# 0xPabloxx/3d-pointcloud-orientation-estimation

Hardware: AMD Instinct MI355X
Metric: clouds/sec fwd+bwd, pointnet_pp_vonMises N=1024 (higher is better)
Workload: dtype f32; 1 GPU; configs[1]: models/pointnet_pp_vonMises.py single-peak KL, N=1024, batch=32 per GPU, fwd+loss+bwd+allreduce+Adam, random-init weights (seed 42), device-side centre sampling; per_gpu_batch=32, global_batch=32, points=1024, parallelism=single, launch=hipGraph(fwd+loss+bwd) + eager all-reduce/Adam (the update clears the gradients)

## Files before the change

### 3d-pointcloud-orientation-estimation_amd/csrc/dw_kernels.hip

```cpp
#include "gemm_smallm.h"
#include "launch.h"
#include "split_prims.h"

namespace pnpp {

template <int DZMODE, int A2MODE, int CT, int KT>
__global__ void __launch_bounds__(256)
dw_kernel(const AOperand dz, const AOperand a2, int M, int Nc, int Kp, int tilesC, int tilesK, int rows_per_split,
          int kp_pad, float *__restrict__ slab, int policy) {
    constexpr int U = 4;
    const int lane = threadIdx.x & 63, l31 = lane & 31, lh = lane >> 5;
    const int gw = blockIdx.x * 4 + (threadIdx.x >> 6);
    const int tiles = tilesC * tilesK;
    const int tile = gw % tiles, split = gw / tiles;
    const int r0 = min(M, split * rows_per_split);
    const int r1 = min(M, r0 + rows_per_split);
    const int c0 = (tile % tilesC) * 32 * CT, k0 = (tile / tilesC) * 32 * KT;

    ChanConst cc[CT], ck[KT];
#pragma unroll
    for (int i = 0; i < CT; ++i) cc[i] = load_chan_const<DZMODE>(dz, c0 + i * 32 + l31, Nc);
#pragma unroll
    for (int j = 0; j < KT; ++j) ck[j] = load_chan_const<A2MODE>(a2, k0 + j * 32 + l31, Kp);

// ... 330 lines not shown
__device__ __forceinline__ void dw_lds_tail(float *__restrict__ o, const f32x16 (&acc)[2][2], int cb, int kb, int Nc, int kp_pad) {
#pragma unroll
    for (int i = 0; i < 2; ++i)
#pragma unroll
        for (int j = 0; j < 2; ++j) {
            const int k = kb + j * 32;
#pragma unroll
            for (int r = 0; r < 16; ++r) {
                const int c = cb + i * 32 + (r & 3) + 8 * (r >> 2);
                if (c < Nc && k < kp_pad) sp_store(o + (size_t)c * kp_pad + k, acc[i][j][r], WT);
            }
        }
}

template <int DZMODE, int A2MODE, bool POLICY>
__device__ __forceinline__ void dw_lds_body(const AOperand &dz, const AOperand &a2, int M, int Nc, int Kp, int tilesC, int tilesK, int rps,
                                            int kp_pad, float *__restrict__ slab, int bx, const bool wt_dw) {
    __shared__ __attribute__((aligned(16))) float Dz[32][128];
    __shared__ __attribute__((aligned(16))) float A2[32][128];
    const int tid = threadIdx.x, lane = tid & 63, wave = __builtin_amdgcn_readfirstlane(tid >> 6);
    const int l31 = lane & 31, lh = lane >> 5;
    const int tiles = tilesC * tilesK;
    const int tile = bx % tiles, split = bx / tiles;
    const int c0 = (tile % tilesC) * 128, k0 = (tile / tilesC) * 128;
    const int r0 = min(M, split * rps), r1 = min(M, r0 + rps);
    const int wc = wave >> 1, wk = wave & 1;
    const int q4 = 4 * (tid & 31), rb = tid >> 5;

    f32x16 acc[2][2];
#pragma unroll
    for (int i = 0; i < 2; ++i)
#pragma unroll
        for (int j = 0; j < 2; ++j)
#pragma unroll
            for (int r = 0; r < 16; ++r) acc[i][j][r] = 0.f;

    RawA nd[4], na[4];
    auto fetch = [&](int m0) {
#pragma unroll
        for (int i = 0; i < 4; ++i) {
            nd[i] = fetch_a4<DZMODE>(dz, m0 + rb + 8 * i, c0 + q4, r1, Nc);
            na[i] = fetch_a4<A2MODE>(a2, m0 + rb + 8 * i, k0 + q4, r1, Kp);
        }
    };
    if (r0 < r1) fetch(r0);
    for (int m0 = r0; m0 < r1; m0 += 32) {
        __syncthreads();
#pragma unroll
        for (int i = 0; i < 4; ++i) {
            float v[4];
            xform_a4<DZMODE>(dz, nd[i], m0 + rb + 8 * i, c0 + q4, r1, Nc, v);
            *reinterpret_cast<float4 *>(&Dz[rb + 8 * i][q4]) = make_float4(v[0], v[1], v[2], v[3]);
            xform_a4<A2MODE>(a2, na[i], m0 + rb + 8 * i, k0 + q4, r1, Kp, v);
            *reinterpret_cast<float4 *>(&A2[rb + 8 * i][q4]) = make_float4(v[0], v[1], v[2], v[3]);
        }
        __syncthreads();
        if (m0 + 32 < r1) fetch(m0 + 32);
        const float *pd = &Dz[lh][wc * 64 + l31], *pa = &A2[lh][wk * 64 + l31];
#pragma unroll 4
        for (int rp = 0; rp < 16; ++rp) {
            const float d0 = pd[rp * 256], d1 = pd[rp * 256 + 32], b0 = pa[rp * 256], b1 = pa[rp * 256 + 32];
            acc[0][0] = __builtin_amdgcn_mfma_f32_32x32x2f32(d0, b0, acc[0][0], 0, 0, 0);
            acc[0][1] = __builtin_amdgcn_mfma_f32_32x32x2f32(d0, b1, acc[0][1], 0, 0, 0);
            acc[1][0] = __builtin_amdgcn_mfma_f32_32x32x2f32(d1, b0, acc[1][0], 0, 0, 0);
            acc[1][1] = __builtin_amdgcn_mfma_f32_32x32x2f32(d1, b1, acc[1][1], 0, 0, 0);
        }
    }
    float *o = slab + (size_t)split * Nc * kp_pad;
    if constexpr (POLICY) {
        if (wt_dw) dw_lds_tail<true>(o, acc, c0 + wc * 64 + 4 * lh, k0 + wk * 64 + l31, Nc, kp_pad);
        else dw_lds_tail<false>(o, acc, c0 + wc * 64 + 4 * lh, k0 + wk * 64 + l31, Nc, kp_pad);
    } else {
        dw_lds_tail<false>(o, acc, c0 + wc * 64 + 4 * lh, k0 + wk * 64 + l31, Nc, kp_pad);
    }
}

template <int DZMODE, int A2MODE>
__global__ void __launch_bounds__(256)
dw_lds_kernel(const AOperand dz, const AOperand a2, int M, int Nc, int Kp, int tilesC, int tilesK, int rps, int kp_pad,
              float *__restrict__ slab) {
    dw_lds_body<DZMODE, A2MODE, false>(dz, a2, M, Nc, Kp, tilesC, tilesK, rps, kp_pad, slab, blockIdx.x, false);
}

template <int EMODE, int A2MODE>
__global__ void __launch_bounds__(256)
da_dw_kernel(const AOperand dzA, const BOperand W, int M, int Nout, int Kd, const Epilogue E, int g1x, int g1, const AOperand a2, int Nc,
             int Kp, int tilesC, int tilesK, int rps, int kp_pad, float *__restrict__ slab) {
    if ((int)blockIdx.x < g1)
        gemm_smallm_body<A_PLAIN, EMODE, false, 4>(dzA, W, M, Nout, Kd, E, blockIdx.x % g1x, blockIdx.x / g1x, g1);
    else
        dw_lds_body<A_PLAIN, A2MODE, true>(dzA, a2, M, Nc, Kp, tilesC, tilesK, rps, kp_pad, slab, blockIdx.x - g1, (E.store_policy & ST_DW_SLABS) != 0);
}

void dw_plan(int M, int Nc, int Kp, int *nsplit, int *kp_pad) {
    const int tilesC = cdiv(Nc, 64), tilesK = cdiv(Kp, 64);
    const int tiles = tilesC * tilesK;
    int split = cdiv(2048, tiles);
    const int max_split = cdiv(M, M <= 4096 ? 32 : 64);
    if (split > max_split) split = max_split;
    if (split > 1024) split = 1024;
    if (split < 1) split = 1;
    *nsplit = split;
    *kp_pad = tilesK * 64;
}

int launch_dw(const AOperand &dz, int Nc, const AOperand &a2, int Kp, int M, float *slab, int nsplit, int kp_pad,
              hipStream_t st) {
    PNPP_REQUIRE(M > 0 && Nc > 0 && Kp > 0 && nsplit > 0, PNPP_ERR_ARG, "dw: non-positive size");
    const int tilesC = cdiv(Nc, 64), tilesK = cdiv(Kp, 64);
    PNPP_REQUIRE(kp_pad == tilesK * 64, PNPP_ERR_ARG, "dw: kp_pad mismatch");
    int rps = cdiv(M, nsplit);
    rps = (rps + 7) & ~7;
    if (M <= 4096 && Nc >= 128 && Kp >= 128 && dz.mode == A_PLAIN && (dz.lda & 3) == 0 && ((uintptr_t)dz.a & 15) == 0 &&
        (a2.mode == A_PLAIN || a2.mode == A_BNRELU || a2.mode == A_CONCAT) &&
        (a2.mode == A_CONCAT || ((a2.lda & 3) == 0 && ((uintptr_t)a2.a & 15) == 0))) {
        const int tc = cdiv(Nc, 128), tk = cdiv(Kp, 128);
        const dim3 grid(tc * tk * nsplit);
        ProfScope ps(st, "dw_lds_kernel<A%d,A%d> M=%d N=%d K=%d split=%d grid=%d", dz.mode, a2.mode, M, Nc, Kp, nsplit, grid.x);
        switch (a2.mode) {
            case A_PLAIN:
                hipLaunchKernelGGL((dw_lds_kernel<A_PLAIN, A_PLAIN>), grid, dim3(256), 0, st, dz, a2, M, Nc, Kp, tc, tk, rps, kp_pad, slab);
                break;
            case A_BNRELU:
                hipLaunchKernelGGL((dw_lds_kernel<A_PLAIN, A_BNRELU>), grid, dim3(256), 0, st, dz, a2, M, Nc, Kp, tc, tk, rps, kp_pad, slab);
                break;
            default:
                hipLaunchKernelGGL((dw_lds_kernel<A_PLAIN, A_CONCAT>), grid, dim3(256), 0, st, dz, a2, M, Nc, Kp, tc, tk, rps, kp_pad, slab);
                break;
        }
        PNPP_CHECK_LAUNCH("dw(lds)");
        return PNPP_OK;
    }
    const int waves = tilesC * tilesK * nsplit;
    const dim3 grid(cdiv(waves, 4)), block(256);
    ProfScope ps(st, "dw_kernel<A%d,A%d> M=%d N=%d K=%d split=%d grid=%dx1", dz.mode, a2.mode, M, Nc, Kp, nsplit, grid.x);
#define PNPP_DW(DM, AM)                                                                                              \
    hipLaunchKernelGGL((dw_kernel<DM, AM, 2, 2>), grid, block, 0, st, dz, a2, M, Nc, Kp, tilesC, tilesK, rps, kp_pad, slab, store_policy()); \
    break;
#define PNPP_DW_BY_A(DM)                         \
    switch (a2.mode) {                           \
        case A_PLAIN: PNPP_DW(DM, A_PLAIN)       \
        case A_BNRELU: PNPP_DW(DM, A_BNRELU)     \
        case A_GATHER: PNPP_DW(DM, A_GATHER)     \
        case A_CONCAT: PNPP_DW(DM, A_CONCAT)     \
        default: set_error("dw: bad A2 mode %d", a2.mode); return PNPP_ERR_ARG; \
    }                                            \
    break;
    switch (dz.mode) {
        case A_PLAIN: PNPP_DW_BY_A(A_PLAIN)
        case A_DZ: PNPP_DW_BY_A(A_DZ)
        case A_DZ_POOL: PNPP_DW_BY_A(A_DZ_POOL)
        default: set_error("dw: bad dZ mode %d", dz.mode); return PNPP_ERR_ARG;
    }
#undef PNPP_DW_BY_A
#undef PNPP_DW
    PNPP_CHECK_LAUNCH("dw");
    return PNPP_OK;
}

bool try_launch_da_dw(const AOperand &dz, const BOperand &Win, int M, int Nout, int Kd, const Epilogue &Ein, int *nslab, const AOperand &a2,
                      int Kp, float *slab, int *nsplit_io, int *kp_pad_io, hipStream_t st, int *rc, float *dw_direct, int dw_ld) {
    *rc = PNPP_OK;
    Epilogue E = Ein;
    E.store_policy = store_policy();
    if (mid_tiles_on() && try_launch_mid_da_dw(dz, Win, M, Nout, Kd, E, nslab, a2, Kp, slab, nsplit_io, kp_pad_io, st, rc, dw_direct, dw_ld))
        return true;
    const int nsplit = *nsplit_io, kp_pad = *kp_pad_io;
    const int Nc = Kd;
    if (!(M > 32 && M <= 4096 && cdiv(M, 32) <= kMaxStatBlocks && dz.mode == A_PLAIN && (dz.lda & 3) == 0 && ((uintptr_t)dz.a & 15) == 0))
        return false;
    if (!(Nc >= 128 && Kp >= 128 && Kd % 4 == 0 && !Win.trans && (E.mode == E_STORE || E.mode == E_MASK_STATS))) return false;
    if (!(a2.mode == A_PLAIN || a2.mode == A_BNRELU || a2.mode == A_CONCAT)) return false;
    if (a2.mode != A_CONCAT && ((a2.lda & 3) != 0 || ((uintptr_t)a2.a & 15) != 0)) return false;
    if (kp_pad != cdiv(Kp, 64) * 64 || nsplit < 1) return false;
    BOperand W = Win;
    if (W.rows <= 0 || W.rows > Kd) W.rows = Kd;
    const int g1x = cdiv(Nout, 32), g1y = cdiv(M, 32), g1 = g1x * g1y;
    const int tc = cdiv(Nc, 128), tk = cdiv(Kp, 128);
    int rps = cdiv(M, nsplit);
    rps = (rps + 7) & ~7;
    const dim3 grid(g1 + tc * tk * nsplit);
    if (nslab) *nslab = g1y;
    ProfScope ps(st, "da_dw_kernel<E%d,A%d> M=%d | dA N=%d K=%d grid=%d | dW N=%d K=%d split=%d grid=%d", E.mode, a2.mode, M, Nout, Kd, g1,
                 Nc, Kp, nsplit, tc * tk * nsplit);
#define PNPP_DADW(EM, AM) \
    hipLaunchKernelGGL((da_dw_kernel<EM, AM>), grid, dim3(256), 0, st, dz, W, M, Nout, Kd, E, g1x, g1, a2, Nc, Kp, tc, tk, rps, kp_pad, slab)
    if (E.mode == E_STORE) {
        if (a2.mode == A_PLAIN) PNPP_DADW(E_STORE, A_PLAIN);
        else if (a2.mode == A_BNRELU) PNPP_DADW(E_STORE, A_BNRELU);
        else PNPP_DADW(E_STORE, A_CONCAT);
    } else {
        if (a2.mode == A_PLAIN) PNPP_DADW(E_MASK_STATS, A_PLAIN);
        else if (a2.mode == A_BNRELU) PNPP_DADW(E_MASK_STATS, A_BNRELU);
        else PNPP_DADW(E_MASK_STATS, A_CONCAT);
    }
#undef PNPP_DADW
    check_launch("da_dw", rc);
    return true;
}

}
```

### 3d-pointcloud-orientation-estimation_amd/csrc/kernels.h

```cpp
#pragma once
#include "common.h"

namespace pnpp {

int launch_knn(const float *new_xyz, const float *xyz, int B, int S, int N, int k, int32_t *idx, hipStream_t st,
               const int32_t *lengths = nullptr);
int launch_knn_centres(const float *xyz, const int32_t *centre, int B, int S, int N, int k, int32_t *idx, float *out_a,
                       float *out_b, hipStream_t st, const int32_t *lengths = nullptr);
int launch_knn_pair(const float *xyz, int B, int N, const int32_t *centre1, int S1, int k1, int32_t *idx1, float *a1, float *b1,
                    const int32_t *centre2, int S2, int k2, int32_t *idx2, float *a2, float *b2, double *mom, hipStream_t st,
                    const int32_t *lengths = nullptr);
int knn_pair_moment_partials(int B, int S1, int N);
size_t knn_pair_moment_doubles(int B, int S1, int N);
int launch_gather_centres(const float *xyz, const int32_t *centre, int B, int N, int S, float *out_a, float *out_b, hipStream_t st);
int launch_scatter_rows_bwd(const float *dout, const int32_t *idx, int B, int N, int C, int M, float *dpoints, hipStream_t st);

enum AMode {
    A_PLAIN = 0,
    A_BNRELU = 1,
    A_GATHER = 2,
    A_CONCAT = 3,
    A_DZ = 4,
    A_DZ_POOL = 5
};
// ... 33 lines not shown
    unsigned long long *rng_counter = nullptr;
    int relu = 0;
    float *y = nullptr;
};

struct Epilogue {
    int mode = E_STORE;
    float *c = nullptr;
    int ldc = 0;
    double *slab = nullptr;
    const float *zp = nullptr;
    const float *scale = nullptr, *shift = nullptr, *mu = nullptr, *istd = nullptr;
    float *dwslab = nullptr;
    int dw_ld = 0;
    float *pool_ext = nullptr;
    int32_t *pool_arg = nullptr;
    const float *pool_gamma = nullptr;
    int store_policy = 0;
    BnTail bn;
};

struct BOperand {
    const float *b = nullptr;
    int ldb = 0;
    int trans = 0;
    int perm_D = -1;
    int rows = 0;
};

struct BnLayer {
    int C = 0;
    const float *bias = nullptr, *gamma = nullptr, *beta = nullptr;
    float *rm = nullptr, *rv = nullptr, *mean = nullptr, *istd = nullptr, *scale = nullptr, *shift = nullptr;
    long long *nbt = nullptr;
};
struct BnGrads { float *dgamma = nullptr, *dbeta = nullptr, *dbias = nullptr; };
struct BnHyper { float momentum = 0.1f, eps = 1e-5f; int training = 0; };
struct StatsView {
    const double *slab = nullptr;
    int nslab = 0;
    const double *count_dev = nullptr, *local = nullptr;
};
struct PoolTail {
    const float *pool_ext = nullptr;
    float *pool_out = nullptr;
    int32_t *pool_arg = nullptr;
    float *origin_a = nullptr, *origin_b = nullptr;
    int G = 0, norigin = 0;
};
struct DzSide { const AOperand *dz = nullptr; int M = 0; float *out = nullptr; };
struct SlabReduceArgs {
    const float *slab;
    int nsplit, Nc, kp_pad, Kvalid, perm_D;
    float *out;
    int ldo;
};

int launch_gemm(const AOperand &A, const BOperand &B, int M, int Nout, int Kd, const Epilogue &E, int *nslab,
                hipStream_t st, int *dw_slabs = nullptr);
bool mid_tiles_on();
bool try_launch_ws(const AOperand &A, const BOperand &B, int M, int Nout, int Kd, const Epilogue &E, int *nslab, hipStream_t st, int *rc,
                   int *dw_slabs);

int matmul_precision();
void set_matmul_precision(int bf16);
bool try_launch_ws_bf16(const AOperand &A, const BOperand &B, int M, int Nout, int Kd, const Epilogue &E, int *nslab, hipStream_t st,
                        int *rc, int *dw_slabs);

int launch_dw(const AOperand &dz, int Nc, const AOperand &a2, int Kp, int M, float *slab, int nsplit, int kp_pad,
              hipStream_t st);
int launch_dz_materialize(const AOperand &dz, int M, int C, float *out, hipStream_t st);
void dw_plan(int M, int Nc, int Kp, int *nsplit, int *kp_pad);
bool delayed_layer0_ok(int C);
int launch_gather_rel_stats(const float *P, const AOperand &geo, const float *W0, int ldw, int M, int C, float *z,
                            double *slab, int *nslab, hipStream_t st);
int scatter_dz_splits(int rows);
int launch_scatter_dz(const AOperand &dz, const AOperand &geo, int B, int Mc, int C, float *G, float *wslab, hipStream_t st);
int dw_xyz_splits(int M);
int launch_dw_xyz(const AOperand &dz, int Nc, const AOperand &a2, int M, float *slab, hipStream_t st);
bool try_launch_fc_dx_dw(const float *dz, const float *w, const float *x, int M, int N, int K, float *dx, float *dw, hipStream_t st,
                         int *rc);
bool try_launch_da_dw(const AOperand &dz, const BOperand &W, int M, int Nout, int Kd, const Epilogue &E, int *nslab, const AOperand &a2,
                      int Kp, float *slab, int *nsplit, int *kp_pad, hipStream_t st, int *rc, float *dw_direct = nullptr, int dw_ld = 0);
bool try_launch_mid_gemm(const AOperand &A, const BOperand &B, int M, int Nout, int Kd, const Epilogue &E, int *nslab, hipStream_t st,
                         int *rc);
bool mid_gemm_pools(const AOperand &A, int M, int Nout, int Kd);
bool try_launch_wsf(const AOperand &A, const BOperand &B, int M, int Nout, int Kd, const Epilogue &E, int *nslab, hipStream_t st, int *rc);
bool wsf_applies(const AOperand &A, const BOperand &B, int M, int Nout, int Kd, const Epilogue &E);
int split_products();
void set_split_products(int on);
int store_policy();
void set_store_policy(int mask);
bool try_launch_wsf3(const AOperand &A, const BOperand &B, int M, int Nout, int Kd, const Epilogue &E, int *nslab, hipStream_t st, int *rc);
bool try_launch_wsd3(const AOperand &A, const BOperand &B, int M, int Nout, int Kd, const Epilogue &E, int *nslab, hipStream_t st, int *rc,
                     int *dw_slabs);
int wsd3_timeouts();
bool try_launch_wsp(const AOperand &A, const BOperand &B, int M, int Nout, int Kd, const Epilogue &E, int *nslab, hipStream_t st, int *rc,
                    int *dw_slabs);
bool try_launch_wsq(const AOperand &A, const BOperand &B, int M, int Nout, int Kd, const Epilogue &E, int *nslab, hipStream_t st, int *rc,
                    int *dw_slabs);
bool try_launch_wsx(const AOperand &dz, const BOperand &W, int M, int C1, int C0, const AOperand &geo, const float *W0, int ldw0,
                    const float *scale0, const float *shift0, float *dwslab, double *stat, int *workers_out, hipStream_t st, int *rc);
size_t wsx_stat_doubles();
bool xyz0_applies(int M, int D, int K, int group_all, int L, const int *C);
size_t xyz0_moment_doubles();
int launch_rel_moments(const AOperand &geo, int M, double *mom, int *nmom, hipStream_t st);
int launch_wsf0(const AOperand &geo, int M, const BOperand &W0, const double *mom, int nmom, const BnLayer &bn0, const BnHyper &h,
                const BOperand &W1, const Epilogue &E, int *nslab, hipStream_t st);
int launch_xyz0_post(const SlabReduceArgs &R1, const double *stat, const BOperand &W0, const BnLayer &bn0, double count, int training,
                     float *dW0, int ld0, const BnGrads &g0, hipStream_t st);
int launch_relu_mask(const float *z, const float *scale, const float *shift, size_t n, int C, uint8_t *out, hipStream_t st);
int launch_xyz0_mask(const AOperand &geo, int M, const float *W0, int ldw0, const float *scale0, const float *shift0, uint8_t *out,
                     hipStream_t st);
unsigned wsx_build_flags();
unsigned wsf_build_flags();
unsigned wsd3_build_flags();
unsigned mid3_build_flags();
unsigned wsp_build_flags();
unsigned wsq_build_flags();
unsigned gemm_build_flags();
unsigned fc_build_flags();
bool try_launch_mid_da_dw(const AOperand &dz, const BOperand &W, int M, int Nout, int Kd, const Epilogue &E, int *nslab, const AOperand &a2,
                          int Kp, float *slab, int *nsplit_out, int *kp_pad_out, hipStream_t st, int *rc, float *dw_direct = nullptr,
                          int dw_ld = 0);
int launch_slab_reduce2(const float *slab1, int nsplit1, int Nc1, int kp_pad1, int Kvalid1, float *out1, int ldo1, const float *slab2,
                        int nsplit2, int Nc2, int kp_pad2, int Kvalid2, float *out2, int ldo2, hipStream_t st);
int launch_slab_reduce(const float *slab, int nsplit, int Nc, int kp_pad, int Kvalid, int perm_D, float *out, int ldo,
                       hipStream_t st);

int launch_bn_finalize_fwd(const StatsView &V, double count, const BnLayer &bn, const BnHyper &h, hipStream_t st,
                           const PoolTail *tail = nullptr);
bool gemm_pools_in_epilogue(const AOperand &A, int M, int Nout, int Kd, int nsample);
struct PooledSource {
    const float *dout = nullptr, *zsel = nullptr, *scale = nullptr, *shift = nullptr;
    int G = 0;
};
int launch_bn_finalize_bwd(const StatsView &V, double count, int training, const BnLayer &bn, float *cst, const BnGrads &g, hipStream_t st,
                           const DzSide &dz = DzSide(), const PooledSource *pooled = nullptr);
int launch_post_gemm(const StatsView &V, double count, int training, const BnLayer &bn, float *cst, const BnGrads &g, const SlabReduceArgs &R,
                     hipStream_t st, const DzSide &dz = DzSide());

bool stats_sync_on();
int launch_slab_sum(const double *slab, int nslab, int C, double count, double *glob, double *local, hipStream_t st);
int stats_exchange(const double *slab, int nslab, int C, double count, hipStream_t st, StatsView *out);
int stats_exchange_inplace(int C, hipStream_t st, StatsView *out);
double *stats_buffer_global();
double *stats_buffer_local();

int pool_fwd_splits(int G, int K, int C);
int launch_pool_fwd(const float *z, const float *scale, const float *shift, int G, int K, int C, float *out, int32_t *arg,
                    hipStream_t st, float *origin_a = nullptr, float *origin_b = nullptr, int norigin = 0, void *part = nullptr,
                    float *zsel = nullptr);
int launch_pool_bwd(const float *dout, const int32_t *arg, const float *z, const float *scale, const float *shift,
                    const float *mean, const float *istd, int G, int K, int C, float *dm, double *slab, int *nslab,
                    hipStream_t st, const float *zsel = nullptr);

int launch_fill_zero(void *p, size_t bytes, hipStream_t st);

int launch_bn_fold_split(const float *w, int Cin, const float *b, const float *gamma, const float *beta, const float *rm, const float *rv,
                         float eps, int C, int ld, unsigned short *wout, float *bout, hipStream_t st);
int infer_target_wgs();

}
```

### 3d-pointcloud-orientation-estimation_amd/pnpp_hip/_lib.py

```python
from __future__ import annotations

import ctypes as C
import os

HERE = os.path.dirname(os.path.abspath(__file__))
LIB_PATH = os.path.join(HERE, "libpnpp_hip.so")

PNPP_MAX_LAYERS = 4
PNPP_OK, PNPP_ERR_ARG, PNPP_ERR_RANGE, PNPP_ERR_LAUNCH, PNPP_ERR_WORKSPACE = 0, -1, -2, -3, -4
NORM_NONE, NORM_BATCH, NORM_LAYER = 0, 1, 2

_fp = C.c_void_p


class SaDesc(C.Structure):
    _fields_ = [("B", C.c_int), ("N", C.c_int), ("S", C.c_int), ("K", C.c_int), ("D", C.c_int), ("L", C.c_int),
                ("C", C.c_int * PNPP_MAX_LAYERS), ("group_all", C.c_int), ("training", C.c_int),
                ("eps", C.c_float), ("momentum", C.c_float)]


_PL = _fp * PNPP_MAX_LAYERS


class SaFwdArgs(C.Structure):
# ... 109 lines not shown
    "pnpp_pn_infer": (_i, [C.POINTER(PnInferDesc), C.POINTER(PnInferArgs), _fp]),
    "pnpp_pt_infer_supported": (_i, [C.POINTER(PtInferDesc)]),
    "pnpp_pt_infer_weights_bytes": (_sz, [C.POINTER(PtInferDesc)]),
    "pnpp_pt_infer_weights_layout": (_i, [C.POINTER(PtInferDesc), _i, _i, C.POINTER(_sz), C.POINTER(_i), C.POINTER(_sz)]),
    "pnpp_pt_infer_fold": (_i, [C.POINTER(PtInferDesc), _i, C.POINTER(PtInferLayerParams), _fp, _fp, _fp, _fp]),
    "pnpp_pt_infer_scratch_bytes": (_sz, [C.POINTER(PtInferDesc)]),
    "pnpp_pt_infer_head": (_i, [C.POINTER(PtInferDesc), _fp, _fp, _fp, _fp, _fp]),
    "pnpp_pt_infer_tail": (_i, [C.POINTER(PtInferDesc), _i, _fp, _fp, _fp, _fp, _fp, _fp, _fp, _fp]),
    "pnpp_pt_infer_pool": (_i, [C.POINTER(PtInferDesc), _fp, _fp, _fp, _i, _fp, _fp]),
    "pnpp_attention_infer": (_i, [_fp, _i, _i, _i, _i, _i, _fp, _fp]),
    "pnpp_attention_infer_supported": (_i, [_i, _i, _i, _i, _i]),
    "pnpp_attention_split_fwd": (_i, [_fp, _i, _i, _i, _i, _i, _fp, _f, _fp, _fp, _fp]),
    "pnpp_attention_split_bwd": (_i, [_fp, _fp, _fp, _fp, _i, _i, _i, _i, _i, _fp, _fp, _f, _fp, _fp, _fp]),
    "pnpp_attention_split_supported": (_i, [_i, _i, _i, _i, _i]),
    "pnpp_attention_fwd_ragged": (_i, [_fp, _i, _i, _i, _fp, _i, _i, _fp, _f, _fp, _fp, _fp]),
    "pnpp_attention_bwd_ragged": (_i, [_fp, _fp, _fp, _fp, _i, _i, _i, _fp, _i, _i, _fp, _fp, _f, _fp, _fp, _fp]),
    "pnpp_attention_split_fwd_ragged": (_i, [_fp, _i, _i, _i, _fp, _i, _i, _fp, _f, _fp, _fp, _fp]),
    "pnpp_attention_split_bwd_ragged": (_i, [_fp, _fp, _fp, _fp, _i, _i, _i, _fp, _i, _i, _fp, _fp, _f, _fp, _fp, _fp]),
    "pnpp_attention_infer_ragged": (_i, [_fp, _i, _i, _i, _fp, _i, _i, _fp, _fp]),
    "pnpp_mean_points_ragged": (_i, [_fp, _i, _i, _fp, _i, _fp, _fp]),
    "pnpp_mean_points_bwd_ragged": (_i, [_fp, _i, _i, _fp, _i, _fp, _fp]),
    "pnpp_pt_infer_head_ragged": (_i, [C.POINTER(PtInferDesc), _fp, _fp, _fp, _fp, _fp, _fp]),
    "pnpp_pt_infer_tail_ragged": (_i, [C.POINTER(PtInferDesc), _fp, _i, _fp, _fp, _fp, _fp, _fp, _fp, _fp, _fp]),
    "pnpp_pt_infer_pool_ragged": (_i, [C.POINTER(PtInferDesc), _fp, _fp, _fp, _fp, _i, _fp, _fp]),
    "pnpp_knn_ragged": (_i, [_fp, _fp, _i, _i, _i, _fp, _i, _fp, _fp]),
    "pnpp_fps_ragged": (_i, [_fp, _i, _i, _fp, _i, _fp, _fp, _fp]),
    "pnpp_ball_query_ragged": (_i, [_fp, _fp, _i, _i, _i, _fp, _f, _i, _fp, _fp]),
    "pnpp_sample_random_ragged": (_i, [_u64, _u64, _i, _i, _fp, _i, _fp, _fp]),
    "pnpp_sample_random_dev_ragged": (_i, [_u64, _fp, _u64, _i, _i, _fp, _i, _fp, _fp]),
    "pnpp_sample_random_dev2_ragged": (_i, [_u64, _fp, _u64, _i, _i, _fp, _i, _fp, _i, _i, _fp, _fp]),
    "pnpp_knn_pair_ragged": (_i, [_fp, _i, _i, _fp, _fp, _i, _i, _fp, _fp, _fp, _i, _i, _fp, _fp, _fp, _fp]),
    "pnpp_sa_group_pair_ragged": (_i, [C.POINTER(SaDesc), C.POINTER(SaDesc), _fp, _fp, _fp, _fp, _fp, _fp, _fp, _fp, _fp]),
    "pnpp_sa_infer_group_pair_ragged": (_i, [C.POINTER(SaDesc), C.POINTER(SaDesc), _fp, _fp, _fp, _fp, _fp, _fp, _fp, _fp, _fp]),
    "pnpp_build_flags": (C.c_uint, []),
    "pnpp_debug_wsd3_timeouts": (_i, []),
    "pnpp_fc_saved_bytes": (_sz, [C.POINTER(FcDesc)]),
    "pnpp_fc_scratch_bytes": (_sz, [C.POINTER(FcDesc)]),
    "pnpp_fc_forward": (_i, [C.POINTER(FcDesc), C.POINTER(FcFwdArgs), _fp]),
    "pnpp_fc_backward": (_i, [C.POINTER(FcDesc), C.POINTER(FcBwdArgs), _fp]),
    "pnpp_vm_head_kl": (_i, [_fp, _fp, _fp, _i, _fp, _fp, _fp, _fp, _fp]),
    "pnpp_vm_fc_head_kl_step": (_i, [_fp, _fp, _fp, _fp, _fp, _i, _i, _fp, _fp, _fp, _fp, _fp]),
    "pnpp_vm_fc_head_kl_step_sample": (_i, [_fp, _fp, _fp, _fp, _fp, _i, _i, _fp, _fp, _fp, _fp, _u64, _fp, _u64, _i, _i, _i, _fp, _i, _i,
                                            _fp, _fp]),
    "pnpp_vm_head_kl_mean": (_i, [_fp, _fp, _fp, _i, _fp, _fp, _fp, _fp, _fp, _fp]),
    "pnpp_vm_head_bwd": (_i, [_fp, _fp, _fp, _i, _fp, _fp]),
    "pnpp_vm_kl_single": (_i, [_fp, _fp, _fp, _fp, _i, _fp, _fp, _fp, _fp]),
    "pnpp_vm_match_loss": (_i, [_fp, _fp, _fp, _fp, _fp, _i, _i, _fp, _fp, _fp, _fp, _fp, _fp]),
    "pnpp_mvm_fc_head_match_step": (_i, [_fp] * 9 + [_i, _i, _i, _f, _f] + [_fp] * 11 + [_u64, _fp, _u64, _i, _i, _i, _fp, _i, _i, _fp, _fp]),
    "pnpp_mvm_head": (_i, [_fp, _fp, _fp, _i, _i, _f, _f, _fp, _fp, _fp, _fp]),
    "pnpp_mvm_head_bwd": (_i, [_fp, _fp, _fp, _fp, _fp, _fp, _fp, _i, _i, _f, _f, _fp, _fp, _fp, _fp]),
    "pnpp_soft_ce": (_i, [_fp, _fp, _i, _i, _fp, _fp, _fp]),
    "pnpp_log_softmax": (_i, [_fp, _i, _i, _fp, _fp]),
    "pnpp_log_softmax_bwd": (_i, [_fp, _fp, _i, _i, _fp, _fp]),
    "pnpp_linear_log_softmax": (_i, [_fp, _fp, _fp, _i, _i, _i, _fp, _fp]),
    "pnpp_nll_loss": (_i, [_fp, _fp, _i, _i, _fp, _fp, _i, _fp]),
    "pnpp_nll_loss_bwd": (_i, [_fp, _fp, _i, _i, _fp, _fp]),
    "pnpp_l2_normalize": (_i, [_fp, _i, _i, _f, _fp, _fp]),
    "pnpp_l2_normalize_bwd": (_i, [_fp, _fp, _i, _i, _f, _fp, _fp]),
    "pnpp_mse": (_i, [_fp, _fp, _sz, _fp, _fp, _fp]),
    "pnpp_mse_rows": (_i, [_fp, _fp, _i, _i, _fp, _fp, _fp]),
    "pnpp_orth_loss": (_i, [_fp, _fp, _i, _i, _fp, _fp, _fp, _fp]),
    "pnpp_proj_probs": (_i, [_fp, _fp, _i, _i, _fp, _fp]),
    "pnpp_proj_probs_bwd": (_i, [_fp, _fp, _fp, _i, _i, _fp, _fp]),
    "pnpp_linear_smallk": (_i, [_fp, _fp, _fp, _i, _i, _i, _fp, _fp]),
    "pnpp_attention_fwd": (_i, [_fp, _i, _i, _i, _i, _i, _fp, _f, _fp, _fp, _fp]),
    "pnpp_attention_dropout_mask": (_i, [_u64, _u64, _i, _i, _i, _f, _fp, _fp, _fp]),
    "pnpp_attention_dropout_mask_dev": (_i, [_u64, _fp, _u64, _i, _i, _i, _f, _fp, _fp, _fp]),
    "pnpp_add_layernorm": (_i, [_fp, _fp, _fp, _fp, _i, _i, _f, _fp, _fp]),
    "pnpp_mean_points": (_i, [_fp, _i, _i, _i, _fp, _fp]),
    "pnpp_linear_smallk_bwd_scratch_bytes": (_sz, [_i, _i]),
    "pnpp_linear_smallk_bwd": (_i, [_fp, _fp, _i, _i, _i, _fp, _fp, _fp, _fp]),
    "pnpp_attention_bwd": (_i, [_fp, _fp, _fp, _fp, _i, _i, _i, _i, _i, _fp, _fp, _f, _fp, _fp, _fp]),
    "pnpp_add_layernorm_bwd_scratch_bytes": (_sz, [_i, _i]),
    "pnpp_add_layernorm_bwd": (_i, [_fp, _fp, _fp, _fp, _i, _i, _f, _fp, _fp, _fp, _fp]),
    "pnpp_mean_points_bwd": (_i, [_fp, _i, _i, _i, _fp, _fp]),
    "pnpp_set_matmul_precision": (_i, [_i]),
    "pnpp_set_stats_exchange": (_i, [STATS_EXCHANGE_FN, C.c_void_p, C.c_void_p, _sz]),
    "pnpp_stats_exchange_enabled": (_i, []),
    "pnpp_get_matmul_precision": (_i, []),
    "pnpp_set_split_products": (_i, [_i]),
    "pnpp_get_split_products": (_i, []),
    "pnpp_set_store_policy": (_i, [_i]),
    "pnpp_get_store_policy": (_i, []),
    "pnpp_adam_step": (_i, [_fp, _fp, _fp, _fp, _sz, _i, _f, _f, _f, _f, _f, _fp]),
    "pnpp_adam_step_zero": (_i, [_fp, _fp, _fp, _fp, _sz, _i, _f, _f, _f, _f, _f, _fp]),
    "pnpp_adam_step_dev": (_i, [_fp, _fp, _fp, _fp, _sz, _fp, _f, _f, _f, _f, _f, _i, _fp]),
    "pnpp_adam_step_clip": (_i, [_fp, _fp, _fp, _fp, _sz, _i, _f, _f, _f, _f, _f, _fp, _f, _i, _fp]),
    "pnpp_adam_step_dev_clip": (_i, [_fp, _fp, _fp, _fp, _sz, _fp, _f, _f, _f, _f, _f, _fp, _f, _i, _fp]),
    "pnpp_sumsq": (_i, [_fp, _sz, _fp, _fp, _sz, _fp]),
    "pnpp_pn_pool_saved_bytes": (_sz, [C.POINTER(PnPoolDesc)]),
    "pnpp_pn_pool_scratch_bytes": (_sz, [C.POINTER(PnPoolDesc)]),
    "pnpp_pn_pool_forward": (_i, [C.POINTER(PnPoolDesc), C.POINTER(PnPoolFwdArgs), _fp]),
    "pnpp_pn_pool_backward": (_i, [C.POINTER(PnPoolDesc), C.POINTER(PnPoolBwdArgs), _fp]),
    "pnpp_pn_pool_saved_route": (_fp, [C.POINTER(PnPoolDesc), _fp]),
    "pnpp_pn_pool_saved_zsel": (_fp, [C.POINTER(PnPoolDesc), _fp]),
    "pnpp_pn_pool_saved_ypre": (_fp, [C.POINTER(PnPoolDesc), _fp]),
    "pnpp_fc_recompute_output": (_i, [C.POINTER(FcDesc), _fp, _fp, _fp, _fp]),
    "pnpp_pn_transform": (_i, [_fp, C.c_int64, C.c_int64, C.c_int64, _fp, _i, _i, _i, _i, _i, _fp, _fp]),
    "pnpp_pn_transform_bwd": (_i, [_fp, C.c_int64, C.c_int64, C.c_int64, _fp, _fp, _i, _i, _i, _i, _i, _fp, _fp, _fp]),
    "pnpp_pn_regularizer": (_i, [_fp, _i, _i, _fp, _fp, _fp]),
    "pnpp_pn_regularizer_bwd": (_i, [_fp, _fp, _fp, _i, _i, _fp, _fp]),
    "pnpp_pn_add_identity": (_i, [_fp, _i, _i, _fp, _fp]),
    "pnpp_pn_concat": (_i, [_fp, _fp, _i, _i, _i, _i, _fp, _fp]),
    "pnpp_pn_concat_bwd": (_i, [_fp, _i, _i, _i, _i, _fp, _fp, _fp]),
    "pnpp_pn_bn_relu": (_i, [_fp, _i, _i, _fp, _fp, _fp, _fp, _fp, _i, _f, _f, _fp, _fp, _fp, _fp]),
    "pnpp_pn_bn_relu_bwd": (_i, [_fp, _fp, _fp, _i, _i, _fp, _fp, _fp, _i, _fp, _fp, _fp, _fp]),
    "pnpp_pn_offsets": (_i, [_fp, _i, _i, _fp, _fp, _fp]),
    "pnpp_pn_pool_saved_bytes_ragged": (_sz, [C.POINTER(PnPoolDesc), _i]),
    "pnpp_pn_pool_scratch_bytes_ragged": (_sz, [C.POINTER(PnPoolDesc), _i]),
    "pnpp_pn_pool_forward_ragged": (_i, [C.POINTER(PnPoolDesc), C.POINTER(PnPoolFwdArgs), _fp, _i, _fp]),
    "pnpp_pn_pool_backward_ragged": (_i, [C.POINTER(PnPoolDesc), C.POINTER(PnPoolBwdArgs), _fp, _i, _fp]),
    "pnpp_pn_transform_ragged": (_i, [_fp, _i, C.c_int64, C.c_int64, C.c_int64, _fp, _fp, _i, _i, _i, _i, _i, _fp, _fp]),
    "pnpp_pn_transform_bwd_ragged": (_i, [_fp, _i, C.c_int64, C.c_int64, C.c_int64, _fp, _fp, _fp, _i, _i, _i, _i, _i, _fp, _fp, _fp]),
    "pnpp_pn_concat_ragged": (_i, [_fp, _fp, _i, _fp, _i, _i, _i, _i, _fp, _fp]),
    "pnpp_pn_concat_bwd_ragged": (_i, [_fp, _fp, _i, _i, _i, _i, _fp, _fp, _fp]),
    "pnpp_pn_infer_ragged": (_i, [C.POINTER(PnInferDesc), C.POINTER(PnInferArgs), _fp, _fp]),
}

_lib = None


class HipExtensionMissing(RuntimeError):
    pass


def lib():
    global _lib
    if _lib is None:
        if not os.path.exists(LIB_PATH):
            raise HipExtensionMissing(
                f"{LIB_PATH} is missing: build it with `python -m pnpp_hip.build` (hipcc, gfx950). "
                "This package has no CPU or PyTorch fallback.")
        try:
            h = C.CDLL(LIB_PATH)
        except OSError as e:
            raise HipExtensionMissing(f"cannot load {LIB_PATH}: {e}") from e
        for name, (res, args) in SIGNATURES.items():
            fn = getattr(h, name)
            fn.restype = res
            fn.argtypes = args
        if h.pnpp_abi_version() != 5:
            raise HipExtensionMissing("libpnpp_hip.so ABI version mismatch; rebuild it")
        _lib = h
    return _lib


def last_error() -> str:
    return lib().pnpp_last_error().decode("utf-8", "replace")


def check(rc: int) -> None:
    if rc == PNPP_OK:
        return
    msg = last_error()
    if rc == PNPP_ERR_ARG:
        raise ValueError(msg)
    raise RuntimeError(msg)
```

### include/pnpp_hip.h

```cpp
#ifndef PNPP_HIP_H
#define PNPP_HIP_H

#include <stddef.h>
#include <stdint.h>

#ifdef __cplusplus
extern "C" {
#endif

typedef enum {
    PNPP_OK = 0,
    PNPP_ERR_ARG = -1,
    PNPP_ERR_RANGE = -2,
    PNPP_ERR_LAUNCH = -3,
    PNPP_ERR_WORKSPACE = -4
} pnpp_status;

const char *pnpp_last_error(void);
int pnpp_abi_version(void);

int pnpp_profile_enable(int on);
int pnpp_profile_report(char *buf_host, size_t buflen);


// ... 140 lines not shown
size_t pnpp_fc_saved_bytes(const pnpp_fc_desc *d);
size_t pnpp_fc_scratch_bytes(const pnpp_fc_desc *d);
int pnpp_fc_forward(const pnpp_fc_desc *d, const pnpp_fc_fwd_args *a, void *stream);
int pnpp_fc_backward(const pnpp_fc_desc *d, const pnpp_fc_bwd_args *a, void *stream);
int pnpp_fc_recompute_output(const pnpp_fc_desc *d, const void *saved, const uint8_t *mask, float *y, void *stream);


int pnpp_vm_head_kl(const float *o, const float *mu_gt, const float *kappa_gt, int B, float *mu, float *kappa,
                    float *loss_vec, float *d_o, void *stream);
int pnpp_vm_fc_head_kl_step(const float *x, const float *w, const float *b, const float *mu_gt, const float *kappa_gt, int B,
                            int K, float *loss_mean, float *dw, float *db, float *dx, void *stream);
int pnpp_vm_fc_head_kl_step_sample(const float *x, const float *w, const float *b, const float *mu_gt, const float *kappa_gt, int B,
                                   int K, float *loss_mean, float *dw, float *db, float *dx, uint64_t seed, uint64_t *stream_id_dev,
                                   uint64_t offset, int Bs, int N1, int npoint1, int32_t *out1, int N2, int npoint2, int32_t *out2,
                                   void *stream);
int pnpp_vm_head_kl_mean(const float *o, const float *mu_gt, const float *kappa_gt, int B, float *mu, float *kappa,
                         float *loss_vec, float *loss_mean, float *d_o_mean, void *stream);
int pnpp_vm_head_bwd(const float *o, const float *dmu, const float *dkappa, int B, float *d_o, void *stream);

int pnpp_vm_kl_single(const float *mu_p, const float *kappa_p, const float *mu_q, const float *kappa_q, int n,
                      float *kl, float *dmu, float *dkappa, void *stream);

int pnpp_vm_match_loss(const float *mu, const float *kappa, const float *w, const float *vm_gt, const int32_t *K_gt,
                       int B, int maxK, float *loss_vec, float *dmu, float *dkappa, float *dw, int32_t *assign,
                       void *stream);

int pnpp_mvm_fc_head_match_step(const float *x, const float *w_pi, const float *b_pi, const float *w_mu, const float *b_mu,
                                const float *w_kappa, const float *b_kappa, const float *vm_gt, const int32_t *K_gt, int B, int K,
                                int maxK, float temp, float kappa_max, float *loss_mean, float *dw_pi, float *db_pi, float *dw_mu,
                                float *db_mu, float *dw_kappa, float *db_kappa, float *dx, float *mu, float *kappa, float *weight,
                                uint64_t seed, uint64_t *stream_id_dev, uint64_t offset, int Bs, int N1, int npoint1, int32_t *out1,
                                int N2, int npoint2, int32_t *out2, void *stream);
int pnpp_mvm_head(const float *pi_raw, const float *mu_raw, const float *kappa_raw, int B, int K, float temp,
                  float kappa_max, float *mu, float *kappa, float *weight, void *stream);
int pnpp_mvm_head_bwd(const float *pi_raw, const float *mu_raw, const float *kappa_raw, const float *weight,
                      const float *dmu, const float *dkappa, const float *dweight, int B, int K, float temp,
                      float kappa_max, float *dpi_raw, float *dmu_raw, float *dkappa_raw, void *stream);

int pnpp_soft_ce(const float *logits, const float *p, int B, int C, float *loss_vec, float *dlogits, void *stream);

int pnpp_log_softmax(const float *x, int M, int C, float *y, void *stream);
int pnpp_log_softmax_bwd(const float *y, const float *dy, int M, int C, float *dx, void *stream);
int pnpp_linear_log_softmax(const float *x, const float *w, const float *b, int M, int K, int C, float *y, void *stream);
int pnpp_nll_loss(const float *logp, const int32_t *target, int M, int C, float *loss_mean, int32_t *bad_targets, int check, void *stream);
int pnpp_nll_loss_bwd(const int32_t *target, const float *grad_loss, int M, int C, float *dlogp, void *stream);

int pnpp_l2_normalize(const float *x, int M, int C, float eps, float *y, void *stream);
int pnpp_l2_normalize_bwd(const float *x, const float *dy, int M, int C, float eps, float *dx, void *stream);
int pnpp_mse(const float *p, const float *t, size_t n, float *loss, float *dp, void *stream);
int pnpp_mse_rows(const float *p, const float *t, int B, int C, float *loss_vec, float *dp, void *stream);
int pnpp_orth_loss(const float *a, const float *b, int B, int C, float *loss, float *da, float *db, void *stream);
int pnpp_proj_probs(const float *vec, const float *dirs, int B, int D, float *probs, void *stream);
int pnpp_proj_probs_bwd(const float *vec, const float *dirs, const float *dprobs, int B, int D, float *dvec, void *stream);

int pnpp_linear_smallk(const float *x, const float *w, const float *b, int M, int K, int N, float *y, void *stream);
int pnpp_attention_fwd(const float *qkv, int B, int N, int n_valid, int H, int head_dim, const uint32_t *mask, float p,
                       float *out, float *lse, void *stream);
int pnpp_attention_dropout_mask(uint64_t seed, uint64_t stream_id, int B, int N, int H, float p, uint32_t *mask,
                                uint32_t *maskT, void *stream);
int pnpp_attention_dropout_mask_dev(uint64_t seed, uint64_t *stream_id_dev, uint64_t offset, int B, int N, int H, float p,
                                    uint32_t *mask, uint32_t *maskT, void *stream);
int pnpp_add_layernorm(const float *x, const float *r, const float *w, const float *b, int M, int E, float eps, float *y,
                       void *stream);
int pnpp_mean_points(const float *x, int B, int N, int E, float *y, void *stream);
size_t pnpp_linear_smallk_bwd_scratch_bytes(int M, int N);
int pnpp_linear_smallk_bwd(const float *x, const float *dy, int M, int K, int N, float *dw, float *db, void *scratch,
                           void *stream);
int pnpp_attention_bwd(const float *qkv, const float *out, const float *d_out, const float *lse, int B, int N, int n_valid, int H,
                       int head_dim, const uint32_t *mask, const uint32_t *maskT, float p, float *dqkv, float *dsum,
                       void *stream);
size_t pnpp_add_layernorm_bwd_scratch_bytes(int M, int E);
int pnpp_add_layernorm_bwd(const float *x, const float *r, const float *w, const float *dy, int M, int E, float eps,
                           float *du, float *dwb, void *scratch, void *stream);
int pnpp_mean_points_bwd(const float *dy, int B, int N, int E, float *dx, void *stream);

int pnpp_set_matmul_precision(int bf16_operands);
int pnpp_get_matmul_precision(void);

int pnpp_set_split_products(int on);
int pnpp_get_split_products(void);

int pnpp_set_store_policy(int mask);
int pnpp_get_store_policy(void);
int pnpp_debug_wsd3_timeouts(void);

typedef int (*pnpp_stats_exchange_fn)(double *buf, size_t n_doubles, void *stream, void *user);
int pnpp_set_stats_exchange(pnpp_stats_exchange_fn fn, void *user, double *buf, size_t buf_doubles);
int pnpp_stats_exchange_enabled(void);

typedef struct {
    int B, N;
    int K, C;
    int relu;
    int training;
    float eps, momentum;
} pnpp_pn_pool_desc;

typedef struct {
    const float *a;
    const float *w, *b;
    const float *gamma, *beta;
    float *rm, *rv;
    int64_t *nbt;
    float *out;
    void *saved;
    void *scratch;
} pnpp_pn_pool_fwd_args;

typedef struct {
    const float *a, *w, *gamma;
    const float *dout;
    const void *saved;
    void *scratch;
    float *da;
    float *dw, *db, *dgamma, *dbeta;
} pnpp_pn_pool_bwd_args;

size_t pnpp_pn_pool_saved_bytes(const pnpp_pn_pool_desc *d);
size_t pnpp_pn_pool_scratch_bytes(const pnpp_pn_pool_desc *d);
int pnpp_pn_pool_forward(const pnpp_pn_pool_desc *d, const pnpp_pn_pool_fwd_args *a, void *stream);
int pnpp_pn_pool_backward(const pnpp_pn_pool_desc *d, const pnpp_pn_pool_bwd_args *a, void *stream);
void *pnpp_pn_pool_saved_route(const pnpp_pn_pool_desc *d, void *saved);
void *pnpp_pn_pool_saved_zsel(const pnpp_pn_pool_desc *d, void *saved);
void *pnpp_pn_pool_saved_ypre(const pnpp_pn_pool_desc *d, void *saved);

int pnpp_pn_transform(const float *x, int64_t sb, int64_t sn, int64_t sd, const float *t, int B, int N, int D, int k, int ldy,
                      float *y, void *stream);
int pnpp_pn_transform_bwd(const float *x, int64_t sb, int64_t sn, int64_t sd, const float *t, const float *dy, int B, int N, int D,
                          int k, int ldy, float *dx, float *dt, void *stream);
int pnpp_pn_regularizer(const float *t, int B, int k, double *norms, float *out, void *stream);
int pnpp_pn_regularizer_bwd(const float *t, const double *norms, const float *dout, int B, int k, float *dt, void *stream);
int pnpp_pn_add_identity(const float *x, int B, int k, float *y, void *stream);
int pnpp_pn_concat(const float *g, const float *pf, int B, int N, int C1, int C2, float *out, void *stream);
int pnpp_pn_concat_bwd(const float *dout, int B, int N, int C1, int C2, float *dg, float *dpf, void *stream);
int pnpp_pn_bn_relu(const float *x, int M, int C, const float *gamma, const float *beta, float *rm, float *rv, int64_t *nbt,
                    int training, float eps, float momentum, float *mean, float *istd, float *y, void *stream);
int pnpp_pn_bn_relu_bwd(const float *x, const float *y, const float *dy, int M, int C, const float *gamma, const float *mean,
                        const float *istd, int training, float *dx, float *dgamma, float *dbeta, void *stream);

int pnpp_pn_offsets(const int32_t *lengths, int B, int N, int32_t *lens_out, int32_t *offs, void *stream);
size_t pnpp_pn_pool_saved_bytes_ragged(const pnpp_pn_pool_desc *d, int M_total);
size_t pnpp_pn_pool_scratch_bytes_ragged(const pnpp_pn_pool_desc *d, int M_total);
int pnpp_pn_pool_forward_ragged(const pnpp_pn_pool_desc *d, const pnpp_pn_pool_fwd_args *a, const int32_t *offs, int M_total, void *stream);
int pnpp_pn_pool_backward_ragged(const pnpp_pn_pool_desc *d, const pnpp_pn_pool_bwd_args *a, const int32_t *offs, int M_total,
                                 void *stream);
int pnpp_pn_transform_ragged(const float *x, int x_packed, int64_t sb, int64_t sn, int64_t sd, const float *t, const int32_t *offs, int B,
                             int N, int D, int k, int ldy, float *y, void *stream);
int pnpp_pn_transform_bwd_ragged(const float *x, int x_packed, int64_t sb, int64_t sn, int64_t sd, const float *t, const float *dy,
                                 const int32_t *offs, int B, int N, int D, int k, int ldy, float *dx, float *dt, void *stream);
int pnpp_pn_concat_ragged(const float *g, const float *pf, int pf_padded, const int32_t *offs, int B, int N, int C1, int C2, float *out,
                          void *stream);
int pnpp_pn_concat_bwd_ragged(const float *dout, const int32_t *offs, int B, int N, int C1, int C2, float *dg, float *dpf, void *stream);

typedef struct {
    const float *xyz;
    const float *points;
    const int32_t *centre_idx;
    const int32_t *neighbour_idx;
    int32_t *idx_out;
    const void *weights;
    float *new_xyz;
    float *out;
} pnpp_sa_infer_args;

int pnpp_sa_infer_supported(const pnpp_sa_desc *d);
size_t pnpp_sa_infer_weights_bytes(const pnpp_sa_desc *d);
// ... 129 lines not shown
```

Before: 61290 clouds/s.

## Add in-place dW path in fused dA/dW kernel writing gradients directly

Adds a path in the fused dA+dW backward kernel for small M (at most 1024) with a BN-ReLU second operand. Each block computes a 32x32 dW tile over all rows, with four waves splitting row chunks and prefetching operands into registers. The four wave partials are reduced through LDS and written straight to the gradient buffer, removing the split-K slab write and its separate reduction pass. In exchange there are fewer, longer dW blocks with less parallelism over rows, which may leave compute units idle. The path is on by default and can be turned off through an environment variable.

```diff
diff --git a/3d-pointcloud-orientation-estimation_amd/csrc/dw_kernels.hip b/3d-pointcloud-orientation-estimation_amd/csrc/dw_kernels.hip
--- a/3d-pointcloud-orientation-estimation_amd/csrc/dw_kernels.hip
+++ b/3d-pointcloud-orientation-estimation_amd/csrc/dw_kernels.hip
@@ -436,12 +436,105 @@
     dw_lds_body<DZMODE, A2MODE, false>(dz, a2, M, Nc, Kp, tilesC, tilesK, rps, kp_pad, slab, blockIdx.x, false);
 }
 
-template <int EMODE, int A2MODE>
+struct DwOut {
+    float *out;
+    int ld;
+};
+
+template <bool WT>
+__device__ __forceinline__ void dw_inplace_tail(const DwOut &O, const float *part, int pstride, int c0, int k0, int Nc, int Kp) {
+#pragma unroll
+    for (int j = 0; j < 4; ++j) {
+        const int e = threadIdx.x + 256 * j, c = c0 + (e >> 5), k = k0 + (e & 31);
+        const float v = (part[e] + part[pstride + e]) + (part[2 * pstride + e] + part[3 * pstride + e]);
+        if (c < Nc && k < Kp) sp_store(O.out + (size_t)c * O.ld + k, v, WT);
+    }
+}
+
+template <int A2MODE, bool FULL>
+__device__ __forceinline__ void dw_inplace_stage(const RawA (&d)[4], const RawA (&a)[4], const ChanConst &cd, const ChanConst (&ca)[4],
+                                                 float *Dz, float *A2, int row, int cq, int kq, int M, int Nc, int Kp, int o) {
+#pragma unroll
+    for (int i = 0; i < 4; ++i) {
+        const bool ok = FULL || row + 8 * i < M;
+        const float dv[4] = {d[i].p.x, d[i].p.y, d[i].p.z, d[i].p.w};
+        const float av[4] = {a[i].p.x, a[i].p.y, a[i].p.z, a[i].p.w};
+        const float aq[4] = {a[i].q.x, a[i].q.y, a[i].q.z, a[i].q.w};
+        float od[4], oa[4];
+#pragma unroll
+        for (int e = 0; e < 4; ++e) {
+            od[e] = xform_a1<A_PLAIN>(make_float2(dv[e], 0.f), cd, FULL ? 0 : cq + e, FULL ? 1 : Nc, ok);
+            oa[e] = xform_a1<A2MODE>(make_float2(av[e], aq[e]), ca[e], FULL ? 0 : kq + e, FULL ? 1 : Kp, ok);
+        }
+        *reinterpret_cast<float4 *>(Dz + o + 256 * i) = make_float4(od[0], od[1], od[2], od[3]);
+        *reinterpret_cast<float4 *>(A2 + o + 256 * i) = make_float4(oa[0], oa[1], oa[2], oa[3]);
+    }
+}
+
+template <int A2MODE>
+__device__ __forceinline__ void dw_inplace_body(const AOperand &dz, const AOperand &a2, int M, int Nc, int Kp, int tilesC, const DwOut &O,
+                                                int bx, const bool wt_dw) {
+    constexpr int IMG = 32 * 32;
+    __shared__ __attribute__((aligned(16))) float img[4 * 2 * IMG];
+    const int tid = threadIdx.x, lane = tid & 63, wave = __builtin_amdgcn_readfirstlane(tid >> 6);
+    const int l31 = lane & 31, lh = lane >> 5;
+    const int c0 = (bx % tilesC) * 32, k0 = (bx / tilesC) * 32;
+    float *Dz = img + wave * 2 * IMG, *A2 = Dz + IMG;
+    const int nchunks = (M + 31) >> 5;
+    const int q4 = 4 * (lane & 7), rb = lane >> 3;
+    const bool inner = c0 + 32 <= Nc && k0 + 32 <= Kp;
+
+    f32x16 acc;
+#pragma unroll
+    for (int r = 0; r < 16; ++r) acc[r] = 0.f;
+
+    constexpr int PF = 4;
+    const ChanConst cd = load_chan_const<A_PLAIN>(dz, c0 + q4, Nc);
+    ChanConst ca[4];
+#pragma unroll
+    for (int e = 0; e < 4; ++e) ca[e] = load_chan_const<A2MODE>(a2, k0 + q4 + e, Kp);
+    RawA nd[PF][4], na[PF][4];
+    auto fetch = [&](RawA(&d)[4], RawA(&a)[4], int c) {
+#pragma unroll
+        for (int i = 0; i < 4; ++i) {
+            d[i] = fetch_a4<A_PLAIN>(dz, c * 32 + rb + 8 * i, c0 + q4, M, Nc);
+            a[i] = fetch_a4<A2MODE>(a2, c * 32 + rb + 8 * i, k0 + q4, M, Kp);
+        }
+    };
+#pragma unroll
+    for (int s = 0; s < PF; ++s)
+        if (wave + 4 * s < nchunks) fetch(nd[s], na[s], wave + 4 * s);
+    for (int cb = wave; cb < nchunks; cb += 4 * PF) {
+#pragma unroll
+        for (int s = 0; s < PF; ++s) {
+            const int c = cb + 4 * s;
+            if (c < nchunks) {
+                if (inner && c * 32 + 32 <= M)
+                    dw_inplace_stage<A2MODE, true>(nd[s], na[s], cd, ca, Dz, A2, c * 32 + rb, c0 + q4, k0 + q4, M, Nc, Kp, rb * 32 + q4);
+                else
+                    dw_inplace_stage<A2MODE, false>(nd[s], na[s], cd, ca, Dz, A2, c * 32 + rb, c0 + q4, k0 + q4, M, Nc, Kp, rb * 32 + q4);
+                if (c + 4 * PF < nchunks) fetch(nd[s], na[s], c + 4 * PF);
+#pragma unroll
+                for (int s2 = 0; s2 < 16; ++s2)
+                    acc = __builtin_amdgcn_mfma_f32_32x32x2f32(Dz[(2 * s2 + lh) * 32 + l31], A2[(2 * s2 + lh) * 32 + l31], acc, 0, 0, 0);
+            }
+        }
+    }
+#pragma unroll
+    for (int r = 0; r < 16; ++r) Dz[((r & 3) + 8 * (r >> 2) + 4 * lh) * 32 + l31] = acc[r];
+    __syncthreads();
+    if (wt_dw) dw_inplace_tail<true>(O, img, 2 * IMG, c0, k0, Nc, Kp);
+    else dw_inplace_tail<false>(O, img, 2 * IMG, c0, k0, Nc, Kp);
+}
+
+template <int EMODE, int A2MODE, bool INPLACE>
 __global__ void __launch_bounds__(256)
 da_dw_kernel(const AOperand dzA, const BOperand W, int M, int Nout, int Kd, const Epilogue E, int g1x, int g1, const AOperand a2, int Nc,
-             int Kp, int tilesC, int tilesK, int rps, int kp_pad, float *__restrict__ slab) {
+             int Kp, int tilesC, int tilesK, int rps, int kp_pad, float *__restrict__ slab, const DwOut O) {
     if ((int)blockIdx.x < g1)
         gemm_smallm_body<A_PLAIN, EMODE, false, 4>(dzA, W, M, Nout, Kd, E, blockIdx.x % g1x, blockIdx.x / g1x, g1);
+    else if constexpr (INPLACE)
+        dw_inplace_body<A2MODE>(dzA, a2, M, Nc, Kp, tilesC, O, blockIdx.x - g1, (E.store_policy & ST_DW_SLABS) != 0);
     else
         dw_lds_body<A_PLAIN, A2MODE, true>(dzA, a2, M, Nc, Kp, tilesC, tilesK, rps, kp_pad, slab, blockIdx.x - g1, (E.store_policy & ST_DW_SLABS) != 0);
 }
@@ -512,6 +605,10 @@
     return PNPP_OK;
 }
 
+static bool g_dw_inplace = true;
+bool dw_inplace_on() { return g_dw_inplace; }
+void set_dw_inplace(bool on) { g_dw_inplace = on; }
+
 bool try_launch_da_dw(const AOperand &dz, const BOperand &Win, int M, int Nout, int Kd, const Epilogue &Ein, int *nslab, const AOperand &a2,
                       int Kp, float *slab, int *nsplit_io, int *kp_pad_io, hipStream_t st, int *rc, float *dw_direct, int dw_ld) {
     *rc = PNPP_OK;
@@ -530,15 +627,29 @@
     BOperand W = Win;
     if (W.rows <= 0 || W.rows > Kd) W.rows = Kd;
     const int g1x = cdiv(Nout, 32), g1y = cdiv(M, 32), g1 = g1x * g1y;
+    if (nslab) *nslab = g1y;
+    if (dw_inplace_on() && dw_direct && M <= 1024 && dw_ld >= Kp && a2.mode == A_BNRELU && (Kp & 3) == 0) {
+        const int tc = cdiv(Nc, 32), g2 = tc * cdiv(Kp, 32);
+        const DwOut O{dw_direct, dw_ld};
+        *nsplit_io = 0;
+        ProfScope ps(st, "da_dw_kernel<E%d,A%d> M=%d | dA N=%d K=%d grid=%d | dW N=%d K=%d split=%d grid=%d", E.mode, a2.mode, M, Nout, Kd,
+                     g1, Nc, Kp, 0, g2);
+        dispatch_mode<E_STORE, E_MASK_STATS>(E.mode, [&](auto em) {
+            hipLaunchKernelGGL((da_dw_kernel<em(), A_BNRELU, true>), dim3(g1 + g2), dim3(256), 0, st, dz, W, M, Nout, Kd, E, g1x, g1, a2, Nc, Kp,
+                               tc, 0, 0, 0, (float *)nullptr, O);
+        });
+        check_launch("da_dw", rc);
+        return true;
+    }
     const int tc = cdiv(Nc, 128), tk = cdiv(Kp, 128);
     int rps = cdiv(M, nsplit);
     rps = (rps + 7) & ~7;
     const dim3 grid(g1 + tc * tk * nsplit);
-    if (nslab) *nslab = g1y;
+    const DwOut O{nullptr, 0};
     ProfScope ps(st, "da_dw_kernel<E%d,A%d> M=%d | dA N=%d K=%d grid=%d | dW N=%d K=%d split=%d grid=%d", E.mode, a2.mode, M, Nout, Kd, g1,
                  Nc, Kp, nsplit, tc * tk * nsplit);
 #define PNPP_DADW(EM, AM) \
-    hipLaunchKernelGGL((da_dw_kernel<EM, AM>), grid, dim3(256), 0, st, dz, W, M, Nout, Kd, E, g1x, g1, a2, Nc, Kp, tc, tk, rps, kp_pad, slab)
+    hipLaunchKernelGGL((da_dw_kernel<EM, AM, false>), grid, dim3(256), 0, st, dz, W, M, Nout, Kd, E, g1x, g1, a2, Nc, Kp, tc, tk, rps, kp_pad, slab, O)
     if (E.mode == E_STORE) {
         if (a2.mode == A_PLAIN) PNPP_DADW(E_STORE, A_PLAIN);
         else if (a2.mode == A_BNRELU) PNPP_DADW(E_STORE, A_BNRELU);
@@ -554,3 +665,9 @@
 }
 
 }
+
+extern "C" int pnpp_set_dw_inplace(int on) {
+    pnpp::set_dw_inplace(on != 0);
+    return PNPP_OK;
+}
+extern "C" int pnpp_get_dw_inplace(void) { return pnpp::dw_inplace_on() ? 1 : 0; }
diff --git a/3d-pointcloud-orientation-estimation_amd/csrc/kernels.h b/3d-pointcloud-orientation-estimation_amd/csrc/kernels.h
--- a/3d-pointcloud-orientation-estimation_amd/csrc/kernels.h
+++ b/3d-pointcloud-orientation-estimation_amd/csrc/kernels.h
@@ -139,6 +139,8 @@
                          int *rc);
 bool try_launch_da_dw(const AOperand &dz, const BOperand &W, int M, int Nout, int Kd, const Epilogue &E, int *nslab, const AOperand &a2,
                       int Kp, float *slab, int *nsplit, int *kp_pad, hipStream_t st, int *rc, float *dw_direct = nullptr, int dw_ld = 0);
+bool dw_inplace_on();
+void set_dw_inplace(bool on);
 bool try_launch_mid_gemm(const AOperand &A, const BOperand &B, int M, int Nout, int Kd, const Epilogue &E, int *nslab, hipStream_t st,
                          int *rc);
 bool mid_gemm_pools(const AOperand &A, int M, int Nout, int Kd);
diff --git a/3d-pointcloud-orientation-estimation_amd/pnpp_hip/_lib.py b/3d-pointcloud-orientation-estimation_amd/pnpp_hip/_lib.py
--- a/3d-pointcloud-orientation-estimation_amd/pnpp_hip/_lib.py
+++ b/3d-pointcloud-orientation-estimation_amd/pnpp_hip/_lib.py
@@ -215,6 +215,8 @@
     "pnpp_get_split_products": (_i, []),
     "pnpp_set_store_policy": (_i, [_i]),
     "pnpp_get_store_policy": (_i, []),
+    "pnpp_set_dw_inplace": (_i, [_i]),
+    "pnpp_get_dw_inplace": (_i, []),
     "pnpp_adam_step": (_i, [_fp, _fp, _fp, _fp, _sz, _i, _f, _f, _f, _f, _f, _fp]),
     "pnpp_adam_step_zero": (_i, [_fp, _fp, _fp, _fp, _sz, _i, _f, _f, _f, _f, _f, _fp]),
     "pnpp_adam_step_dev": (_i, [_fp, _fp, _fp, _fp, _sz, _fp, _f, _f, _f, _f, _f, _i, _fp]),
@@ -274,6 +276,8 @@
             fn.argtypes = args
         if h.pnpp_abi_version() != 5:
             raise HipExtensionMissing("libpnpp_hip.so ABI version mismatch; rebuild it")
+        if os.environ.get("PNPP_DW_INPLACE") is not None:
+            h.pnpp_set_dw_inplace(1 if os.environ["PNPP_DW_INPLACE"].strip() not in ("", "0") else 0)
         _lib = h
     return _lib
 
diff --git a/include/pnpp_hip.h b/include/pnpp_hip.h
--- a/include/pnpp_hip.h
+++ b/include/pnpp_hip.h
@@ -246,6 +246,9 @@
 
 int pnpp_set_store_policy(int mask);
 int pnpp_get_store_policy(void);
+
+int pnpp_set_dw_inplace(int on);
+int pnpp_get_dw_inplace(void);
 int pnpp_debug_wsd3_timeouts(void);
 
 typedef int (*pnpp_stats_exchange_fn)(double *buf, size_t n_doubles, void *stream, void *user);
```

Result: no change. 61660 clouds/s, median of 6 (+0.6%).
